# shrubb/latent-pose-reenactment

Hardware: AMD Instinct MI355X
Metric: train-step images/sec at 256x256 bs=8 (higher is better)
Workload: dtype mixed 16-bit MFMA operands, fp32 accumulate, fp32 activations / weights / optimizer state; 1 GPU; default.yaml meta-training step (configs[2]): ResNeXt50 identity encoder over 8 frames + MobileNetV2 pose encoder (both trained, forward + backward on hand-written gfx950 kernels), G, D with the 98000x512 label embedding, VGG19/VGGFace/featmat/adversarial/dis_embed/dice criterions, Adam, EMA; image_size=256, per_gpu_batch=8, global_batch=8, parallelism=dp1, precision_mode=default assignment (LP_PREC=f16), padding=zero, launch_mode=hipgraph

## Files before the change

include/lp_hip.h:

```cpp
#ifndef LP_HIP_H
#define LP_HIP_H
#include <stdint.h>
#ifdef __cplusplus
extern "C" {
#endif

#define LP_OK 0
#define LP_ERR_ARG (-1)
#define LP_ERR_UNSUPPORTED (-2)
#define LP_ERR_HIP (-3)

#define LP_PREC_BF16 0
#define LP_PREC_BF16X3 1
#define LP_PREC_F16 2

const char* lp_last_error(void);
int lp_abi_version(void);

int lp_pack_weights(const float* w, uint16_t* hi, uint16_t* lo, int Cout, int Cin, int T, int RowsP, int ColsP, int mode, int f16,
                    void* stream);
int lp_pack_desc_bytes(void);
int lp_pack_weights_batch(const void* table, int num_entries, long long total_chunks, void* stream);
int lp_pack_pair_desc_bytes(void);
int lp_pack_weights_pairs(const void* table, int num_entries, long long total_tiles, void* stream);
// ... 89 lines not shown
                    int frozen_stats, float* amax_slots, void* stream);

long long lp_bn_train_stats_workspace_bytes(long long P, int C);
int lp_bn_train_stats(const float* y, const float* gamma, const float* beta, float eps, float momentum, float* running_mean,
                      float* running_var, float* mean, float* rstd, float* scale, float* shift, float* workspace,
                      long long P, int C, void* stream);

int lp_gconv16_fwd(const uint16_t* a_hi, const uint16_t* a_lo, const uint16_t* w_hi, const uint16_t* w_lo, float* y, const float* alpha2,
                   int N, int H, int W, int C, int CP, int prec, float* amax_slots, void* stream);
int lp_gconv16_fwd_stats(const uint16_t* a_hi, const uint16_t* a_lo, const uint16_t* w_hi, const uint16_t* w_lo, float* y, const float* alpha2,
                         int N, int H, int W, int C, int CP, int prec, float* amax_slots, float* stats, long long stats_capacity_floats,
                         int* stats_rows, void* stream);
int lp_gconv16_fwd_planes(const uint16_t* a_hi, const uint16_t* a_lo, const uint16_t* w_hi, const uint16_t* w_lo, float* y, uint16_t* o_hi,
                          uint16_t* o_lo, const float* alpha2, int N, int H, int W, int C, int CP, int group_size, int prec, float* amax_slots,
                          float* stats, long long stats_capacity_floats, int* stats_rows, void* stream);
long long lp_gconv_wgrad_workspace_bytes(int C, int splits);
int lp_gconv16_wgrad(const uint16_t* a_hi, const uint16_t* a_lo, const uint16_t* dy_hi, const uint16_t* dy_lo, float* dw, float* workspace,
                     int N, int H, int W, int C, int group_size, int splits, int prec, const float* out_scale, void* stream);
int lp_pack_grouped(const float* w, uint16_t* hi, uint16_t* lo, int C, int group_size, int CP, int mode, int f16, void* stream);
int lp_im2col_planes(const float* x, uint16_t* hi, uint16_t* lo, int N, int C, int H, int W, int ksize, int stride, int pad, int prec,
                     void* stream);
int lp_bn_relu_maxpool_fwd(const float* y, const float* scale, const float* shift, float* out, uint16_t* hi, uint16_t* lo,
                           unsigned char* idx, int N, int H, int W, int C, int prec, void* stream);
int lp_maxpool_bwd(const float* dout, const unsigned char* idx, float* dA, int N, int H, int W, int C, void* stream);
int lp_bn_add_act(const float* y, const float* scale, const float* shift, const float* res, const float* res_scale, const float* res_shift,
                  float* out, uint16_t* hi, uint16_t* lo, long long P, int C, int relu, int prec, void* stream);
int lp_bn_add_act_planes(const float* y, const float* scale, const float* shift, const uint16_t* res_hi, const uint16_t* res_lo, float* out,
                         uint16_t* hi, uint16_t* lo, long long P, int C, int relu, int prec, void* stream);
int lp_bn_add_act16(const uint16_t* y16, const float* scale, const float* shift, const float* res, const float* res_scale,
                    const float* res_shift, float* out, uint16_t* hi, long long P, int C, int relu, void* stream);
// ... 147 lines not shown
```

latent_pose_reenactment_amd/_lib.py:

```python
import ctypes
import os

import torch

_HERE = os.path.dirname(os.path.abspath(__file__))
LIB_PATH = os.environ.get('LP_LIB_OVERRIDE') or os.path.join(_HERE, 'liblp_hip.so')

PREC_BF16 = 0
PREC_BF16X3 = 1
PREC_F16 = 2

_vp, _i, _f, _ll = ctypes.c_void_p, ctypes.c_int, ctypes.c_float, ctypes.c_longlong

SIGNATURES = {
    'lp_last_error': (ctypes.c_char_p, []),
    'lp_abi_version': (_i, []),
    'lp_pack_weights': (_i, [_vp, _vp, _vp, _i, _i, _i, _i, _i, _i, _i, _vp]),
    'lp_pack_desc_bytes': (_i, []),
    'lp_pack_weights_batch': (_i, [_vp, _i, _ll, _vp]),
    'lp_pack_pair_desc_bytes': (_i, []),
    'lp_pack_weights_pairs': (_i, [_vp, _i, _ll, _vp]),
    'lp_act_pack': (_i, [_vp, _vp, _vp, _i, _vp, _vp, _i, _i, _i, _i, _vp, _vp, _i, _i, _vp, _vp]),
    'lp_amax_slots': (_i, []),
    'lp_amax_slot_stride': (_i, []),
    'lp_amax_blocks': (_i, []),
    'lp_amax_partial': (_i, [_vp, _ll, _vp, _vp]),
    'lp_conv16_fwd': (_i, [_vp] * 9 + [_i] * 11 + [_vp, _vp, _vp, _i, _vp, _ll, _vp, _vp]),
    'lp_conv16_fwd_workspace_bytes': (_ll, [_i] * 5),
    'lp_conv16_fwd_stats': (_i, [_vp] * 9 + [_i] * 11 + [_vp, _vp, _vp, _i, _vp, _ll, _vp, _vp, _ll, _vp, _vp]),
    'lp_conv16_stats_floats': (_ll, [_i] * 4),
    'lp_norm_stats_finalize': (_i, [_vp, _i, _vp, _vp, _i, _f, _f, _vp, _vp, _vp, _vp, _vp, _vp, _i, _i, _vp]),
    'lp_gconv16_fwd_stats': (_i, [_vp] * 6 + [_i] * 6 + [_vp, _vp, _ll, _vp, _vp]),
    'lp_gconv16_fwd_planes': (_i, [_vp] * 8 + [_i] * 7 + [_vp, _vp, _ll, _vp, _vp]),
    'lp_conv_wgrad_workspace_bytes': (_ll, [_i, _i, _i, _i]),
    'lp_conv16_wgrad': (_i, [_vp] * 6 + [_i] * 9 + [_vp, _i, _vp, _vp, _vp, _vp]),
    'lp_conv_wgrad_dot_blocks': (_i, [_i] * 3),
    'lp_thin_conv_supported': (_i, [_i] * 4),
    'lp_thin_conv_fwd': (_i, [_vp] * 6 + [_i] * 9 + [_vp, _i, _vp]),
    'lp_thin_conv_emits_planes': (_i, [_i] * 5),
    'lp_thin_wgrad_supported': (_i, [_i] * 5),
    'lp_thin_wgrad_has_dbias': (_i, [_i] * 2),
    'lp_thin_wgrad': (_i, [_vp] * 6 + [_i] * 8 + [_vp, _vp]),
    'lp_linear_fwd': (_i, [_vp, _vp, _vp, _vp, _vp, _i, _i, _i, _vp]),
    'lp_linear_bwd_workspace_bytes': (_ll, [_i, _i, _i]),
    'lp_linear_bwd': (_i, [_vp] * 8 + [_i, _i, _i, _vp]),
    'lp_grid_crop_fwd': (_i, [_vp, _vp, _vp, _i, _i, _i, _i, _i, _i, _vp]),
    'lp_grid_crop_bwd': (_i, [_vp, _vp, _vp, _i, _i, _i, _i, _i, _i, _vp]),
    'lp_stem_conv_s2': (_i, [_vp, _vp, _vp, _i, _i, _i, _i, _vp]),
# ... 108 lines not shown
_lib = None


class LpError(RuntimeError):
    pass


def lib():
    global _lib
    if _lib is None:
        if not os.path.exists(LIB_PATH):
            raise LpError(f'{LIB_PATH} is missing: run `python -m latent_pose_reenactment_amd.build` '
                          '(or __graft_entry__.build()); there is no fallback path')
        l = ctypes.CDLL(LIB_PATH)
        for name, (res, args) in SIGNATURES.items():
            fn = getattr(l, name)
            fn.restype, fn.argtypes = res, args
        _lib = l
    return _lib


def check(rc, what):
    if rc != 0:
        msg = lib().lp_last_error()
        raise LpError(f'{what} failed (rc={rc}): {msg.decode() if msg else ""}')
```

latent_pose_reenactment_amd/csrc/gconv_rows.hip:

```cpp
#include "lp_common.h"
#include "conv_common.h"
#include "lp_hip.h"
#include "lp_internal.h"
#include <stdlib.h>

#if defined(__HIP_DEVICE_COMPILE__)
#pragma clang attribute push(__attribute__((target("no-packed-fp32-ops"))), apply_to = function)
#endif

static __device__ __attribute__((aligned(64))) unsigned int gr_zero_page[16];

static __device__ __forceinline__ void gr_barrier() {
    __builtin_amdgcn_fence(__ATOMIC_RELEASE, "workgroup");
    __builtin_amdgcn_s_barrier();
    __builtin_amdgcn_fence(__ATOMIC_ACQUIRE, "workgroup");
}
static __device__ __forceinline__ float gr_shfl_xor(float v, int lane, int o) {
    return __builtin_bit_cast(float, __builtin_amdgcn_ds_bpermute((lane ^ o) << 2, __builtin_bit_cast(int, v)));
}

struct GconvRowsParams {
    const uint16_t* a_hi; const uint16_t* a_lo; const uint16_t* w_hi; const uint16_t* w_lo;
    float* y; uint16_t* o_hi; uint16_t* o_lo; const float* alpha2; float* amax; float* stats;
    int N, H, W, C, CP;
    int tiles_x, tiles_y, ntiles;
    int nblk, wgs, xcd;
};

namespace gr {
constexpr int TH = 4, TW = 16, HH = TH + 2, HW = TW + 2, HALO_PX = HH * HW;
constexpr int PIECES = (HALO_PX * 128 + 1023) / 1024;
constexpr int PLANE = PIECES * 1024;
constexpr int KIT = (PIECES + 3) / 4;
__host__ __device__ constexpr int key(int hp) { return ((hp >> 1) & 3) << 1; }
}

template <int PREC>
__global__ __launch_bounds__(256, PREC == LP_PREC_BF16X3 ? 2 : 4) void gconv_rows_kernel(GconvRowsParams p) {
    using namespace gr;
    constexpr bool SPLIT = (PREC == LP_PREC_BF16X3), F16 = (PREC == LP_PREC_F16);
    constexpr int BUF = PLANE * (SPLIT ? 2 : 1);
    extern __shared__ __attribute__((aligned(16))) unsigned char smem[];

    const int lane = (int)threadIdx.x & 63;
    const int wave = __builtin_amdgcn_readfirstlane((int)threadIdx.x >> 6);
    const int kb = lane >> 4, px = lane & 15;

    int blk, t0, tstep, tend;
    {
        const int id = (int)blockIdx.x;
        if (p.xcd) {
            const int x = id & 7, j = id >> 3, per = (p.ntiles + 7) >> 3;
            blk = j % p.nblk;
            tstep = p.wgs >> 3;
// ... 17 lines not shown
        wlo[s] = (s16x8_t){0, 0, 0, 0, 0, 0, 0, 0};
        if (tap < 9) {
            const size_t off = ((size_t)tap * p.CP + co0 + 16 * wave + px) * 64 + 16 * wave + 8 * (kb & 1);
            whi[s] = *(const s16x8_t*)(p.w_hi + off);
            if (SPLIT) wlo[s] = *(const s16x8_t*)(p.w_lo + off);
        }
    }
    const float alpha = p.alpha2 ? *p.alpha2 : 1.f;

    int r_off[TH][5];
#pragma unroll
    for (int s = 0; s < 5; ++s) {
        const int tap = min(2 * s + (lane >> 5), 8);
#pragma unroll
        for (int r = 0; r < TH; ++r) {
            const int hp = (r + tap / 3) * HW + px + tap % 3;
            r_off[r][s] = hp * 128 + (((2 * wave + (kb & 1)) ^ key(hp)) << 4);
        }
    }

    int d_hy[KIT], d_hx[KIT], d_c[KIT];
#pragma unroll
    for (int k = 0; k < KIT; ++k) {
        const int hp = (4 * k + wave) * 8 + (lane >> 3);
        d_hy[k] = hp < HALO_PX ? hp / HW : -(1 << 20);
        d_hx[k] = hp % HW;
        d_c[k] = co0 + (((lane & 7) ^ key(hp)) << 3);
    }
    const uint16_t* zero16 = (const uint16_t*)gr_zero_page;
    const unsigned lds0 = (unsigned)__builtin_amdgcn_readfirstlane((int)(unsigned)(uintptr_t)smem);
    auto decode = [&](int t, int& n, int& y0, int& x0) {
        x0 = (t % p.tiles_x) * TW; t /= p.tiles_x;
        y0 = (t % p.tiles_y) * TH; n = t / p.tiles_y;
    };
    auto issue = [&](int t, int buf) {
        int n, y0, x0;
        decode(t, n, y0, x0);
#pragma unroll
        for (int k = 0; k < KIT; ++k) {
            const int q = 4 * k + wave;
            if (q < PIECES) {
                const int iy = y0 - 1 + d_hy[k], ix = x0 - 1 + d_hx[k];
                const bool ok = iy >= 0 && iy < p.H && ix >= 0 && ix < p.W;
                const size_t off = ok ? ((size_t)(n * p.H + iy) * p.W + ix) * p.C + d_c[k] : 0;
                const unsigned d = lds0 + (unsigned)(buf * BUF + q * 1024);
                lp_glds16(ok ? (p.a_hi + off) : zero16, d);
                if (SPLIT) lp_glds16(ok ? (p.a_lo + off) : zero16, d + PLANE);
            }
        }
    };

    float am = 0.f;
    issue(t0, 0);
    int buf = 0;
    for (int t = t0; t < tend; t += tstep, buf ^= 1) {
        lp_wait_vm0();
        gr_barrier();
// ... 28 lines not shown
            const int oy = y0 + r, ox = x0 + px;
            float4 v;
            v.x = fmaf(acc[0], alpha, 0.f); v.y = fmaf(acc[1], alpha, 0.f); v.z = fmaf(acc[2], alpha, 0.f); v.w = fmaf(acc[3], alpha, 0.f);
            if (p.stats) {
                const float o4[4] = {v.x, v.y, v.z, v.w};
#pragma unroll
                for (int k = 0; k < 4; ++k)
#pragma unroll
                    for (int j = 0; j < 4; ++j) {
                        const float xv = __builtin_bit_cast(float, __builtin_amdgcn_ds_bpermute(((lane & 48) | (4 * k + (px & 3))) << 2, __builtin_bit_cast(int, o4[j])));
                        if (r == 0 && k == 0) st_ref[j] = xv;
                        const float d = xv - st_ref[j];
                        st_d[j] += d; st_q[j] = fmaf(d, d, st_q[j]);
                    }
            }
            if (oy < p.H && ox < p.W) {
                const size_t e = (((size_t)n * p.H + oy) * p.W + ox) * p.C + co0 + 16 * wave + 4 * kb;
                if (p.y) *(float4*)(p.y + e) = v;
                am = lp_amax4(am, v);
                if (p.o_hi) {
                    const float o[4] = {v.x, v.y, v.z, v.w};
                    ushort4 oh, ol;
                    uint16_t* ohp = (uint16_t*)&oh; uint16_t* olp = (uint16_t*)&ol;
#pragma unroll
                    for (int j = 0; j < 4; ++j) {
                        ohp[j] = lp_f32_to_op16<F16>(o[j]);
                        if (SPLIT) olp[j] = lp_f32_to_op16<false>(o[j] - lp_op16_to_f32<false>(ohp[j]));
                    }
                    *(ushort4*)(p.o_hi + e) = oh;
                    if (SPLIT) *(ushort4*)(p.o_lo + e) = ol;
                }
            }
// ... 2 lines not shown
            float cnt = 16.f, mean[4], m2[4];
#pragma unroll
            for (int j = 0; j < 4; ++j) { mean[j] = st_ref[j] + st_d[j] / cnt; m2[j] = fmaxf(st_q[j] - st_d[j] * st_d[j] / cnt, 0.f); }
#pragma unroll
            for (int o = 1; o < 4; o <<= 1) {
#pragma unroll
                for (int j = 0; j < 4; ++j) {
                    const float mb = gr_shfl_xor(mean[j], lane, o), qb = gr_shfl_xor(m2[j], lane, o);
                    const float d = mb - mean[j];
                    mean[j] = fmaf(d, 0.5f, mean[j]); m2[j] += qb + d * d * (cnt * 0.5f);
                }
                cnt *= 2.f;
            }
            if (px == 0) {
                const int ty = y0 >> 2;
                const int rb = ((n * (p.tiles_y >> 2) + (ty >> 2)) * p.tiles_x + (x0 >> 4)) * 4 + (ty & 3);
                float* o = p.stats + ((size_t)rb * p.C + co0 + 16 * wave + 4 * kb) * 3;
#pragma unroll
                for (int j = 0; j < 4; ++j) { o[j * 3 + 0] = cnt; o[j * 3 + 1] = mean[j]; o[j * 3 + 2] = m2[j]; }
            }
        }
    }
    if (p.amax) lp_amax_commit(am, p.amax, blockIdx.x);
}

#if defined(__HIP_DEVICE_COMPILE__)
#pragma clang attribute pop
#endif

int lp_gconv_rows_launch(Conv16Params& c, int group_size, int prec, hipStream_t s) {
    static const int mode = getenv("LP_GCONV_ROWS") ? atoi(getenv("LP_GCONV_ROWS")) : 1;
    static const int wgs_cap = getenv("LP_GCONV_ROWS_WGS") ? atoi(getenv("LP_GCONV_ROWS_WGS")) : 0;
    if (mode == 0 || !(group_size == 4 || group_size == 8 || group_size == 16)) return 0;
    if (prec != LP_PREC_BF16 && prec != LP_PREC_BF16X3 && prec != LP_PREC_F16) return 0;
    const bool exact = (c.W % gr::TW == 0) && (c.H % gr::TH == 0);
    if (mode != 2 && !exact) return 0;
    const bool patches = (c.W % 16 == 0) && (c.H % 16 == 0);
    if (c.stats && !patches && (c.H * c.W) % 64 == 0) return 0;
    GconvRowsParams p;
    p.a_hi = c.a_hi; p.a_lo = c.a_lo; p.w_hi = c.w_hi; p.w_lo = c.w_lo; p.y = c.y; p.o_hi = c.o_hi; p.o_lo = c.o_lo; p.alpha2 = c.alpha2; p.amax = c.amax;
    p.N = c.N; p.H = c.H; p.W = c.W; p.C = c.Cout; p.CP = c.CoutP;
    p.tiles_x = (c.W + gr::TW - 1) / gr::TW; p.tiles_y = (c.H + gr::TH - 1) / gr::TH; p.ntiles = c.N * p.tiles_x * p.tiles_y;
    p.nblk = c.Cout / 64;
    c.stats_rows = 0;
    if (c.stats) {
        const long long rows = (long long)c.N * (c.H * c.W / 64);
        if (patches && rows * c.Cout * 3 <= c.stats_cap) c.stats_rows = c.H * c.W / 64; else c.stats = nullptr;
    }
    p.stats = c.stats;
    const int occ = prec == LP_PREC_BF16X3 ? 2 : 4;
    static int cus = 0;
    if (!cus) { int dev = 0; if (hipGetDevice(&dev) != hipSuccess || hipDeviceGetAttribute(&cus, hipDeviceAttributeMultiprocessorCount, dev) != hipSuccess || cus < 1) cus = 256; }
    int wgs = (cus * occ + p.nblk - 1) / p.nblk;
    if (wgs_cap > 0 && wgs > wgs_cap) wgs = wgs_cap;
    if (wgs > p.ntiles) wgs = p.ntiles;
    p.xcd = (wgs >= 8 && p.ntiles >= 16) ? 1 : 0;
    if (p.xcd) wgs &= ~7;
    p.wgs = wgs;
    const dim3 grid((unsigned)(p.nblk * wgs));
    const size_t lds = 2 * gr::PLANE * (prec == LP_PREC_BF16X3 ? 2 : 1);
    if (prec == LP_PREC_BF16X3) hipLaunchKernelGGL(gconv_rows_kernel<LP_PREC_BF16X3>, grid, dim3(256), lds, s, p);
    else if (prec == LP_PREC_F16) hipLaunchKernelGGL(gconv_rows_kernel<LP_PREC_F16>, grid, dim3(256), lds, s, p);
    else hipLaunchKernelGGL(gconv_rows_kernel<LP_PREC_BF16>, grid, dim3(256), lds, s, p);
    const int rc = lp_check_launch("gconv_rows");
    return rc ? rc : 1;
}
```

latent_pose_reenactment_amd/embedders/resnext_hip.py:

```python
import os

import torch

from latent_pose_reenactment_amd import hipops as ops
from latent_pose_reenactment_amd import streams as _streams
from latent_pose_reenactment_amd._lib import PREC_BF16X3, PREC_F16


class _BN:
    __slots__ = ('mean', 'rstd', 'scale', 'shift')

    def __init__(self, mean, rstd, scale, shift):
        self.mean, self.rstd, self.scale, self.shift = mean, rstd, scale, shift


def supported(n: int, h: int, w: int) -> bool:
    return h % 32 == 0 and w % 32 == 0 and h >= 128 and w >= 128 and n % 4 == 0 and n >= 8


Y16 = os.environ.get('LP_E_Y16', '1') != '0'
RES16 = os.environ.get('LP_E_RES16', '1') != '0'
MASK16 = os.environ.get('LP_E_MASK16', '1') != '0'


# ... 23 lines not shown
def _bn_relu_planes(y, st, prec):
    if isinstance(y, ops.Act16):
        return ops.bn_act16(y, st.scale, st.shift)
    return ops.act_pack(y, pro=4, scale=st.scale, shift=st.shift, prec=prec)


def bn_state(y, st, gamma, beta, m, counters):
    if m.track_running_stats:
        counters.append(m.num_batches_tracked)
    rm, rv = (m.running_mean, m.running_var) if m.track_running_stats else (None, None)
    if st is not None:
        return _BN(*ops.norm_stats_finalize(st, 1, gamma.shape[0], gamma, beta, m.eps, running_mean=rm, running_var=rv, momentum=m.momentum))
    if isinstance(y, ops.Act16):
        y = ops.y16_to_f32(y)
    return _BN(*ops.bn_train_stats(y, gamma, beta, rm, rv, m.momentum, m.eps))


def _wgrad1x1(a16, d16, prec, bias_grad=False):
    return ops.conv_wgrad16(ops.flat16(a16), ops.flat16(d16), ksize=1, prec=prec, bias_grad=bias_grad, kind='wgrad1x1')


class ResNeXtFunction(torch.autograd.Function):

    @staticmethod
    def forward(ctx, net, x, *params):
        prec = net.prec
        train = net.training
        need_grad = any(ctx.needs_input_grad[2:])
        if ctx.needs_input_grad[1]:
            raise RuntimeError('the HIP encoder does not differentiate with respect to its input frames (detach them)')
# ... 34 lines not shown
            y16 = Y16 and p1 == p2 == p3 == PREC_F16
            assert not (y16 and nprec != PREC_F16), 'an fp16 block must be followed by fp16 blocks (lp_bn_add_act16 writes fp16 planes)'
            xin, xin16 = out, out16
            _, h, w, _ = xin16.hi.shape
            y1, cs = _conv1x1(xin16, packs[bname + '.conv1.weight'][0], p1, stats=True, y16=y16)
            y1 = _yview(y1, (n, h, w, width))
            st1 = bn(y1, bname + '.bn1', cs)
            a1 = _bn_relu_planes(y1, st1, p2)
            if stride == 1:
                if y16:
                    _, y2, cs = ops.gconv16(a1, packs[bname + '.conv2.weight'][0], prec=p2, stats=True, want_y=False, out16=True)
                else:
                    y2, cs = ops.gconv16(a1, packs[bname + '.conv2.weight'][0], prec=p2, stats=True)
                ho, wo = h, w
            else:
                y2, cs = ops.subsample2(ops.gconv16(a1, packs[bname + '.conv2.weight'][0], prec=p2)), None
                ho, wo = y2.shape[1], y2.shape[2]
            st2 = bn(y2, bname + '.bn2', cs)
            a2 = _bn_relu_planes(y2, st2, p3)
            y3, cs = _conv1x1(a2, packs[bname + '.conv3.weight'][0], p3, stats=True, y16=y16)
            y3 = _yview(y3, (n, ho, wo, cout))
            st3 = bn(y3, bname + '.bn3', cs)
            xd16 = yd = std = None
            if down:
                xd16 = ops.subsample2_16(xin16) if stride == 2 else xin16
                yd, cs = _conv1x1(xd16, packs[bname + '.downsample.0.weight'][0], p1, stats=True)
                yd = yd.view(n, ho, wo, cout)
                std = bn(yd, bname + '.downsample.1', cs)
                need_f32 = bi + 1 >= nblk or not (net._hip_blocks[bi + 1][5] or planes_res[bi + 1])
                out, out16 = ops.bn_add_act(y3, st3.scale, st3.shift, yd, std.scale, std.shift, relu=True, prec=nprec, want_out=need_f32 or not MASK16)
            elif planes_res[bi]:
# ... 47 lines not shown
            else:
                grads[key] = fn(*operands)

        p16, (hl, wl, cl), (fh, fw) = ctx.head
        dl16 = ops.act_pack(d_logits.contiguous().view(1, fh, fw, -1), prec=prec, grad=True)
        dw, db = ops.conv_wgrad16(p16, dl16, ksize=1, prec=prec, bias_grad=True)
        grads['fc.weight'], grads['fc.bias'] = dw.view(par['fc.weight'].shape), db
        d_pooled = ops.conv16(dl16, packs['fc.weight'][1], ksize=1, prec=prec).view(n, cl)
        d_out = ops.spatial_mean_bwd(d_pooled, hl, wl)
        for (bname, cin, width, cout, stride, down), sv in zip(reversed(net._hip_blocks), reversed(ctx.blocks)):
            xin16, y1, st1, a1, y2, st2, a2, y3, st3, xd16, yd, std, out, (h, w, ho, wo), (p1, p2, p3) = sv
            d16, g = bn_bwd(d_out, y3, st3, bname + '.bn3', p3, mask_mode=2, mask_src=out, want_g=not down)
            wgrad(bname + '.conv3.weight', lambda a, d, k=bname + '.conv3.weight', p=p3: _wgrad1x1(a, d, p).view(par[k].shape), a2, d16)
            dA2 = _conv1x1(d16, packs[bname + '.conv3.weight'][1], p3).view(n, ho, wo, width)
            d16, _ = bn_bwd(dA2, y2, st2, bname + '.bn2', p2)
            if stride == 2:
                d16 = ops.zero_stuff2_16(d16, h, w)
            cg = par[bname + '.conv2.weight'].shape[1]
            wgrad(bname + '.conv2.weight', lambda a, d, cg=cg, p=p2: ops.gconv_wgrad16(a, d, cg, prec=p), a1, d16)
            dA1 = ops.gconv16(d16, packs[bname + '.conv2.weight'][1], prec=p2)
            d16, _ = bn_bwd(dA1, y1, st1, bname + '.bn1', p1)
            wgrad(bname + '.conv1.weight', lambda a, d, k=bname + '.conv1.weight', p=p1: _wgrad1x1(a, d, p).view(par[k].shape), xin16, d16)
            if down:
                dd16, _ = bn_bwd(d_out, yd, std, bname + '.downsample.1', p1, mask_mode=2, mask_src=out)
                wgrad(bname + '.downsample.0.weight', lambda a, d, k=bname + '.downsample.0.weight', p=p1: _wgrad1x1(a, d, p).view(par[k].shape), xd16, dd16)
                d_xd = _conv1x1(dd16, packs[bname + '.downsample.0.weight'][1], p1)
                if stride == 2:
                    d_xin = _conv1x1(d16, packs[bname + '.conv1.weight'][1], p1).view(n, h, w, cin)
                    ops.add_strided2(d_xin, d_xd.view(n, ho, wo, cin))
                else:
                    d_xin = _conv1x1(d16, packs[bname + '.conv1.weight'][1], p1, res=d_xd).view(n, h, w, cin)
            else:
                d_xin = _conv1x1(d16, packs[bname + '.conv1.weight'][1], p1, res=g).view(n, h, w, cin)
            d_out = d_xin
        prec = net.prec
# ... 11 lines not shown
```

latent_pose_reenactment_amd/hipops.py:

```python
import os
from typing import NamedTuple, Optional, Tuple

import torch

from . import _lib
from ._lib import PREC_BF16, PREC_BF16X3, PREC_F16, check
from .dataloaders.synthetic_voxceleb2_stickmen import PARTS

Tensor = torch.Tensor


def _stream():
    return torch.cuda.current_stream().cuda_stream


PROFILE = None


class _Timed:
    def __init__(self, kind, flops, tag=None, nbytes=0.0, mm=1):
        self.mm = mm
        self.rw = tuple(nbytes) if isinstance(nbytes, tuple) else None
        self.kind, self.flops, self.tag, self.nbytes = kind, flops, tag, (sum(nbytes) if isinstance(nbytes, tuple) else nbytes)

# ... 1820 lines not shown
                                     mask_mode, mptr, _p(g), float(act_hi), int(frozen), _p(_amax_attach(dx, amax)), _stream()),
          'lp_norm_act_bwd')
    return dx, dgb[0], dgb[1], g


def pack_grouped(w: Tensor, mode: int, prec: int) -> WeightPack:
    _chk(w, 'w')
    c, cg = w.shape[0], w.shape[1]
    cp = _round_up(c, 128)
    hi = torch.empty((9, cp, 64), dtype=torch.int16, device=w.device)
    lo = torch.empty_like(hi) if prec == PREC_BF16X3 else None
    check(_lib.lib().lp_pack_grouped(w.data_ptr(), hi.data_ptr(), _p(lo), c, cg, cp, mode, _f16(prec), _stream()), 'lp_pack_grouped')
    return WeightPack(hi, lo, c, cg, cp, 64, 9)


def gconv16(a: Act16, pack: WeightPack, *, prec: int, amax: bool = False, stats: bool = False, want_y: bool = True, out16: bool = False):
    n, h, w = a.nhw
    c = a.c
    assert c == pack.rows and a.hi.shape[3] == c, (a.hi.shape, pack.rows)
    assert want_y or (out16 and not amax)
    dev = a.hi.device
    y = torch.empty((n, h, w, c), dtype=torch.float32, device=dev) if want_y else None
    o_hi = o_lo = None
    if out16:
        o_hi, o_lo = _alloc16(n, h, w, c, prec, dev)
    slots = _amax_attach(y, amax and prec == PREC_F16) if y is not None else None
    st_buf, st_rows, st_cap = None, None, 0
    if stats:
        import ctypes
        st_cap = _lib.lib().lp_conv16_stats_floats(n, h, w, c)
        st_buf = torch.empty(st_cap, dtype=torch.float32, device=dev)
        st_rows = ctypes.c_int(0)
    pl = 4 if prec == PREC_BF16X3 else 2
    nbytes = n * h * w * c * (pl + (4 if want_y else 0) + (pl if out16 else 0)) + pack.hi.numel() * pl
    with _Timed('gconv', 2.0 * n * h * w * c * pack.cols * 9, (n, h, w, pack.cols, c, 3, 0, 0), nbytes, mm=3 if prec == PREC_BF16X3 else 1):
        check(_lib.lib().lp_gconv16_fwd_planes(a.hi.data_ptr(), _p(a.lo), pack.hi.data_ptr(), _p(pack.lo), _p(y), _p(o_hi), _p(o_lo), _p(a.inv),
                                               n, h, w, c, pack.rows_p, pack.cols, prec, _p(slots), _p(st_buf), st_cap,
                                               None if st_rows is None else ctypes.addressof(st_rows), _stream()), 'lp_gconv16_fwd')
    out = (y,) if not out16 else (y, Act16(o_hi, o_lo, c, None))
    if stats:
        out = out + ((ConvStats(st_buf, st_rows.value, n) if st_rows.value > 0 else None),)
    return out[0] if len(out) == 1 else out


def bn_act16(y16: Act16, scale: Tensor, shift: Tensor, relu: bool = True) -> Act16:
    c = y16.c
    assert y16.lo is None and y16.inv is None and y16.hi.shape[-1] == c and c % 8 == 0
    hi = torch.empty_like(y16.hi)
    check(_lib.lib().lp_bn_act16(y16.hi.data_ptr(), scale.data_ptr(), shift.data_ptr(), hi.data_ptr(), y16.hi.numel() // c, c, int(relu),
                                 _stream()), 'lp_bn_act16')
    return Act16(hi, None, c, None)


# ... 267 lines not shown
```

Before: 204.9 images/s.

## Add native stride-2 grouped conv forward and polyphase dgrad for ResNeXt

Adds a stride-2 variant of the row-tiled grouped 3x3 conv kernel that computes only the subsampled outputs, with fused BN stats, instead of running a full-resolution conv and subsampling afterwards. It also adds a polyphase stride-2 data-gradient kernel that reads the low-resolution gradient directly, so the zero-stuffed full-resolution gradient is no longer convolved. The point is to remove the wasted MACs (about 3/4) and memory traffic in the stride-2 blocks of the ResNeXt encoder. The cost is more kernel code and a halo layout with even/odd column splitting, plus lower occupancy bounds for the S=2 kernel.

```diff
diff --git a/include/lp_hip.h b/include/lp_hip.h
--- a/include/lp_hip.h
+++ b/include/lp_hip.h
@@ -127,6 +127,12 @@
 int lp_gconv16_fwd_planes(const uint16_t* a_hi, const uint16_t* a_lo, const uint16_t* w_hi, const uint16_t* w_lo, float* y, uint16_t* o_hi,
                           uint16_t* o_lo, const float* alpha2, int N, int H, int W, int C, int CP, int group_size, int prec, float* amax_slots,
                           float* stats, long long stats_capacity_floats, int* stats_rows, void* stream);
+int lp_gconv16_s2_covered(int H, int W, int group_size);
+int lp_gconv16_s2_fwd_planes(const uint16_t* a_hi, const uint16_t* a_lo, const uint16_t* w_hi, const uint16_t* w_lo, float* y, uint16_t* o_hi,
+                             uint16_t* o_lo, const float* alpha2, int N, int H, int W, int C, int CP, int group_size, int prec,
+                             float* amax_slots, float* stats, long long stats_capacity_floats, int* stats_rows, void* stream);
+int lp_gconv16_s2_dgrad(const uint16_t* d_hi, const uint16_t* d_lo, const uint16_t* w_hi, const uint16_t* w_lo, float* dx, const float* alpha2,
+                        int N, int H, int W, int C, int CP, int group_size, int prec, float* amax_slots, void* stream);
 long long lp_gconv_wgrad_workspace_bytes(int C, int splits);
 int lp_gconv16_wgrad(const uint16_t* a_hi, const uint16_t* a_lo, const uint16_t* dy_hi, const uint16_t* dy_lo, float* dw, float* workspace,
                      int N, int H, int W, int C, int group_size, int splits, int prec, const float* out_scale, void* stream);
diff --git a/latent_pose_reenactment_amd/_lib.py b/latent_pose_reenactment_amd/_lib.py
--- a/latent_pose_reenactment_amd/_lib.py
+++ b/latent_pose_reenactment_amd/_lib.py
@@ -32,6 +32,9 @@
     'lp_norm_stats_finalize': (_i, [_vp, _i, _vp, _vp, _i, _f, _f, _vp, _vp, _vp, _vp, _vp, _vp, _i, _i, _vp]),
     'lp_gconv16_fwd_stats': (_i, [_vp] * 6 + [_i] * 6 + [_vp, _vp, _ll, _vp, _vp]),
     'lp_gconv16_fwd_planes': (_i, [_vp] * 8 + [_i] * 7 + [_vp, _vp, _ll, _vp, _vp]),
+    'lp_gconv16_s2_covered': (_i, [_i] * 3),
+    'lp_gconv16_s2_fwd_planes': (_i, [_vp] * 8 + [_i] * 7 + [_vp, _vp, _ll, _vp, _vp]),
+    'lp_gconv16_s2_dgrad': (_i, [_vp] * 6 + [_i] * 7 + [_vp, _vp]),
     'lp_conv_wgrad_workspace_bytes': (_ll, [_i, _i, _i, _i]),
     'lp_conv16_wgrad': (_i, [_vp] * 6 + [_i] * 9 + [_vp, _i, _vp, _vp, _vp, _vp]),
     'lp_conv_wgrad_dot_blocks': (_i, [_i] * 3),
@@ -170,6 +173,8 @@
                           '(or __graft_entry__.build()); there is no fallback path')
         l = ctypes.CDLL(LIB_PATH)
         for name, (res, args) in SIGNATURES.items():
+            if os.environ.get('LP_LIB_OVERRIDE') and not hasattr(l, name):
+                continue
             fn = getattr(l, name)
             fn.restype, fn.argtypes = res, args
         _lib = l
diff --git a/latent_pose_reenactment_amd/csrc/gconv_rows.hip b/latent_pose_reenactment_amd/csrc/gconv_rows.hip
--- a/latent_pose_reenactment_amd/csrc/gconv_rows.hip
+++ b/latent_pose_reenactment_amd/csrc/gconv_rows.hip
@@ -23,21 +23,28 @@
     const uint16_t* a_hi; const uint16_t* a_lo; const uint16_t* w_hi; const uint16_t* w_lo;
     float* y; uint16_t* o_hi; uint16_t* o_lo; const float* alpha2; float* amax; float* stats;
     int N, H, W, C, CP;
+    int Ho, Wo;
     int tiles_x, tiles_y, ntiles;
     int nblk, wgs, xcd;
 };
 
 namespace gr {
-constexpr int TH = 4, TW = 16, HH = TH + 2, HW = TW + 2, HALO_PX = HH * HW;
-constexpr int PIECES = (HALO_PX * 128 + 1023) / 1024;
-constexpr int PLANE = PIECES * 1024;
-constexpr int KIT = (PIECES + 3) / 4;
+constexpr int TH = 4, TW = 16;
+template <int S> struct Geo {
+    static constexpr int HH = S * (TH - 1) + 3, HW = S * (TW - 1) + 3, HALO_PX = HH * HW;
+    static constexpr int EV = TW + 1;
+    static constexpr int PIECES = (HALO_PX * 128 + 1023) / 1024;
+    static constexpr int PLANE = PIECES * 1024;
+    static constexpr int KIT = (PIECES + 3) / 4;
+};
 __host__ __device__ constexpr int key(int hp) { return ((hp >> 1) & 3) << 1; }
 }
 
-template <int PREC>
-__global__ __launch_bounds__(256, PREC == LP_PREC_BF16X3 ? 2 : 4) void gconv_rows_kernel(GconvRowsParams p) {
+template <int PREC, int S>
+__global__ __launch_bounds__(256, (PREC == LP_PREC_BF16X3 ? 2 : 4) / S) void gconv_rows_kernel(GconvRowsParams p) {
     using namespace gr;
+    using G = Geo<S>;
+    constexpr int HW = G::HW, HALO_PX = G::HALO_PX, PIECES = G::PIECES, PLANE = G::PLANE, KIT = G::KIT;
     constexpr bool SPLIT = (PREC == LP_PREC_BF16X3), F16 = (PREC == LP_PREC_F16);
     constexpr int BUF = PLANE * (SPLIT ? 2 : 1);
     extern __shared__ __attribute__((aligned(16))) unsigned char smem[];
@@ -85,7 +92,8 @@
         const int tap = min(2 * s + (lane >> 5), 8);
 #pragma unroll
         for (int r = 0; r < TH; ++r) {
-            const int hp = (r + tap / 3) * HW + px + tap % 3;
+            const int dy = tap / 3, dx = tap % 3;
+            const int hp = S == 1 ? (r + dy) * HW + px + dx : (2 * r + dy) * HW + (dx == 1 ? G::EV + px : px + (dx >> 1));
             r_off[r][s] = hp * 128 + (((2 * wave + (kb & 1)) ^ key(hp)) << 4);
         }
     }
@@ -95,7 +103,7 @@
     for (int k = 0; k < KIT; ++k) {
         const int hp = (4 * k + wave) * 8 + (lane >> 3);
         d_hy[k] = hp < HALO_PX ? hp / HW : -(1 << 20);
-        d_hx[k] = hp % HW;
+        d_hx[k] = S == 1 ? hp % HW : (hp % HW < G::EV ? 2 * (hp % HW) : 2 * (hp % HW - G::EV) + 1);
         d_c[k] = co0 + (((lane & 7) ^ key(hp)) << 3);
     }
     const uint16_t* zero16 = (const uint16_t*)gr_zero_page;
@@ -111,7 +119,7 @@
         for (int k = 0; k < KIT; ++k) {
             const int q = 4 * k + wave;
             if (q < PIECES) {
-                const int iy = y0 - 1 + d_hy[k], ix = x0 - 1 + d_hx[k];
+                const int iy = S * y0 - 1 + d_hy[k], ix = S * x0 - 1 + d_hx[k];
                 const bool ok = iy >= 0 && iy < p.H && ix >= 0 && ix < p.W;
                 const size_t off = ok ? ((size_t)(n * p.H + iy) * p.W + ix) * p.C + d_c[k] : 0;
                 const unsigned d = lds0 + (unsigned)(buf * BUF + q * 1024);
@@ -170,8 +178,8 @@
                         st_d[j] += d; st_q[j] = fmaf(d, d, st_q[j]);
                     }
             }
-            if (oy < p.H && ox < p.W) {
-                const size_t e = (((size_t)n * p.H + oy) * p.W + ox) * p.C + co0 + 16 * wave + 4 * kb;
+            if (oy < p.Ho && ox < p.Wo) {
+                const size_t e = (((size_t)n * p.Ho + oy) * p.Wo + ox) * p.C + co0 + 16 * wave + 4 * kb;
                 if (p.y) *(float4*)(p.y + e) = v;
                 am = lp_amax4(am, v);
                 if (p.o_hi) {
@@ -204,10 +212,162 @@
             }
             if (px == 0) {
                 const int ty = y0 >> 2;
-                const int rb = ((n * (p.tiles_y >> 2) + (ty >> 2)) * p.tiles_x + (x0 >> 4)) * 4 + (ty & 3);
+                const int rb = S == 1 ? ((n * (p.tiles_y >> 2) + (ty >> 2)) * p.tiles_x + (x0 >> 4)) * 4 + (ty & 3) : t;
                 float* o = p.stats + ((size_t)rb * p.C + co0 + 16 * wave + 4 * kb) * 3;
 #pragma unroll
                 for (int j = 0; j < 4; ++j) { o[j * 3 + 0] = cnt; o[j * 3 + 1] = mean[j]; o[j * 3 + 2] = m2[j]; }
+            }
+        }
+    }
+    if (p.amax) lp_amax_commit(am, p.amax, blockIdx.x);
+}
+
+struct GconvS2DgradParams {
+    const uint16_t* d_hi; const uint16_t* d_lo; const uint16_t* w_hi; const uint16_t* w_lo;
+    float* dx; const float* alpha2; float* amax;
+    int N, H, W, Ho, Wo, C, CP;
+    int tiles_x, tiles_y, ntiles;
+    int nblk, wgs, xcd;
+};
+
+namespace gd {
+constexpr int TH = 4, TW = 16, HH = TH + 1, HW = TW + 1, HALO_PX = HH * HW;
+constexpr int PIECES = (HALO_PX * 128 + 1023) / 1024;
+constexpr int PLANE = PIECES * 1024;
+constexpr int KIT = (PIECES + 3) / 4;
+}
+
+template <int PREC>
+__global__ __launch_bounds__(256, PREC == LP_PREC_BF16X3 ? 2 : 4) void gconv_rows_s2_dgrad_kernel(GconvS2DgradParams p) {
+    using namespace gd;
+    constexpr bool SPLIT = (PREC == LP_PREC_BF16X3), F16 = (PREC == LP_PREC_F16);
+    constexpr int BUF = PLANE * (SPLIT ? 2 : 1);
+    extern __shared__ __attribute__((aligned(16))) unsigned char smem[];
+
+    const int lane = (int)threadIdx.x & 63;
+    const int wave = __builtin_amdgcn_readfirstlane((int)threadIdx.x >> 6);
+    const int kb = lane >> 4, px = lane & 15;
+
+    int blk, t0, tstep, tend;
+    {
+        const int id = (int)blockIdx.x;
+        if (p.xcd) {
+            const int x = id & 7, j = id >> 3, per = (p.ntiles + 7) >> 3;
+            blk = j % p.nblk;
+            tstep = p.wgs >> 3;
+            t0 = x * per + j / p.nblk;
+            tend = min(x * per + per, p.ntiles);
+        } else {
+            blk = id % p.nblk;
+            tstep = p.wgs;
+            t0 = id / p.nblk;
+            tend = p.ntiles;
+        }
+    }
+    if (t0 >= tend) return;
+    const int co0 = blk * 64;
+
+    s16x8_t whi[5], wlo[5];
+#pragma unroll
+    for (int s = 0; s < 5; ++s) {
+        const int tap = 2 * s + (lane >> 5);
+        whi[s] = (s16x8_t){0, 0, 0, 0, 0, 0, 0, 0};
+        wlo[s] = (s16x8_t){0, 0, 0, 0, 0, 0, 0, 0};
+        if (tap < 9) {
+            const size_t off = ((size_t)tap * p.CP + co0 + 16 * wave + px) * 64 + 16 * wave + 8 * (kb & 1);
+            whi[s] = *(const s16x8_t*)(p.w_hi + off);
+            if (SPLIT) wlo[s] = *(const s16x8_t*)(p.w_lo + off);
+        }
+    }
+    const float alpha = p.alpha2 ? *p.alpha2 : 1.f;
+
+    int r_off[HH][2];
+#pragma unroll
+    for (int hy = 0; hy < HH; ++hy)
+#pragma unroll
+        for (int ex = 0; ex < 2; ++ex) {
+            const int hp = hy * HW + px + ex;
+            r_off[hy][ex] = hp * 128 + (((2 * wave + (kb & 1)) ^ gr::key(hp)) << 4);
+        }
+
+    int d_hy[KIT], d_hx[KIT], d_c[KIT];
+#pragma unroll
+    for (int k = 0; k < KIT; ++k) {
+        const int hp = (4 * k + wave) * 8 + (lane >> 3);
+        d_hy[k] = hp < HALO_PX ? hp / HW : (1 << 20);
+        d_hx[k] = hp % HW;
+        d_c[k] = co0 + (((lane & 7) ^ gr::key(hp)) << 3);
+    }
+    const uint16_t* zero16 = (const uint16_t*)gr_zero_page;
+    const unsigned lds0 = (unsigned)__builtin_amdgcn_readfirstlane((int)(unsigned)(uintptr_t)smem);
+    auto decode = [&](int t, int& n, int& y0, int& x0) {
+        x0 = (t % p.tiles_x) * TW; t /= p.tiles_x;
+        y0 = (t % p.tiles_y) * TH; n = t / p.tiles_y;
+    };
+    auto issue = [&](int t, int buf) {
+        int n, y0, x0;
+        decode(t, n, y0, x0);
+#pragma unroll
+        for (int k = 0; k < KIT; ++k) {
+            const int q = 4 * k + wave;
+            if (q < PIECES) {
+                const int sy = y0 + d_hy[k], sx = x0 + d_hx[k];
+                const bool ok = sy < p.Ho && sx < p.Wo;
+                const size_t off = ok ? ((size_t)(n * p.Ho + sy) * p.Wo + sx) * p.C + d_c[k] : 0;
+                const unsigned d = lds0 + (unsigned)(buf * BUF + q * 1024);
+                lp_glds16(ok ? (p.d_hi + off) : zero16, d);
+                if (SPLIT) lp_glds16(ok ? (p.d_lo + off) : zero16, d + PLANE);
+            }
+        }
+    };
+
+    float am = 0.f;
+    issue(t0, 0);
+    int buf = 0;
+    for (int t = t0; t < tend; t += tstep, buf ^= 1) {
+        lp_wait_vm0();
+        gr_barrier();
+        if (t + tstep < tend) issue(t + tstep, buf ^ 1);
+        int n, y0, x0;
+        decode(t, n, y0, x0);
+        const unsigned char* Hb = smem + buf * BUF;
+#pragma unroll
+        for (int a = 0; a < TH; ++a) {
+            int lhalf = lane >> 5;
+            asm volatile("" : "+v"(lhalf));
+            s16x8_t fh[2][2], fl[2][2];
+#pragma unroll
+            for (int ey = 0; ey < 2; ++ey)
+#pragma unroll
+                for (int ex = 0; ex < 2; ++ex) {
+                    fh[ey][ex] = *(const s16x8_t*)(Hb + r_off[a + ey][ex]);
+                    if (SPLIT) fl[ey][ex] = *(const s16x8_t*)(Hb + PLANE + r_off[a + ey][ex]);
+                }
+#pragma unroll
+            for (int ph = 0; ph < 4; ++ph) {
+                const int pa = ph >> 1, pb = ph & 1;
+                f32x4_t acc = (f32x4_t){0.f, 0.f, 0.f, 0.f};
+#pragma unroll
+                for (int tap = 0; tap < 9; ++tap) {
+                    const int dy = tap / 3, dx = tap % 3;
+                    if ((dy == 1) != (pa == 0) || (dx == 1) != (pb == 0)) continue;
+                    const int ey = dy == 2, ex = dx == 2, s = tap >> 1, h = tap & 1;
+                    const s16x8_t zero = (s16x8_t){0, 0, 0, 0, 0, 0, 0, 0};
+                    const s16x8_t mh = (lhalf == h) ? whi[s] : zero;
+                    if (SPLIT) {
+                        const s16x8_t ml = (lhalf == h) ? wlo[s] : zero;
+                        acc = mfma16t<false>(mh, fl[ey][ex], acc);
+                        acc = mfma16t<false>(ml, fh[ey][ex], acc);
+                    }
+                    acc = mfma16t<F16>(mh, fh[ey][ex], acc);
+                }
+                const int iy = 2 * (y0 + a) + pa, ix = 2 * (x0 + px) + pb;
+                float4 v;
+                v.x = fmaf(acc[0], alpha, 0.f); v.y = fmaf(acc[1], alpha, 0.f); v.z = fmaf(acc[2], alpha, 0.f); v.w = fmaf(acc[3], alpha, 0.f);
+                if (iy < p.H && ix < p.W) {
+                    *(float4*)(p.dx + (((size_t)n * p.H + iy) * p.W + ix) * p.C + co0 + 16 * wave + 4 * kb) = v;
+                    am = lp_amax4(am, v);
+                }
             }
         }
     }
@@ -218,9 +378,26 @@
 #pragma clang attribute pop
 #endif
 
+static int gr_mode() {
+    static const int mode = getenv("LP_GCONV_ROWS") ? atoi(getenv("LP_GCONV_ROWS")) : 1;
+    return mode;
+}
+
+static int gr_workgroups(int nblk, int ntiles, int occ, int& xcd) {
+    static const int wgs_cap = getenv("LP_GCONV_ROWS_WGS") ? atoi(getenv("LP_GCONV_ROWS_WGS")) : 0;
+    static int cus = 0;
+    if (!cus) { int dev = 0; if (hipGetDevice(&dev) != hipSuccess || hipDeviceGetAttribute(&cus, hipDeviceAttributeMultiprocessorCount, dev) != hipSuccess || cus < 1) cus = 256; }
+    int wgs = (cus * occ + nblk - 1) / nblk;
+    if (wgs_cap > 0 && wgs > wgs_cap) wgs = wgs_cap;
+    if (wgs > ntiles) wgs = ntiles;
+    xcd = (wgs >= 8 && ntiles >= 16) ? 1 : 0;
+    if (xcd) wgs &= ~7;
+    return wgs;
+}
+
 int lp_gconv_rows_launch(Conv16Params& c, int group_size, int prec, hipStream_t s) {
-    static const int mode = getenv("LP_GCONV_ROWS") ? atoi(getenv("LP_GCONV_ROWS")) : 1;
-    static const int wgs_cap = getenv("LP_GCONV_ROWS_WGS") ? atoi(getenv("LP_GCONV_ROWS_WGS")) : 0;
+    using G = gr::Geo<1>;
+    const int mode = gr_mode();
     if (mode == 0 || !(group_size == 4 || group_size == 8 || group_size == 16)) return 0;
     if (prec != LP_PREC_BF16 && prec != LP_PREC_BF16X3 && prec != LP_PREC_F16) return 0;
     const bool exact = (c.W % gr::TW == 0) && (c.H % gr::TH == 0);
@@ -229,7 +406,7 @@
     if (c.stats && !patches && (c.H * c.W) % 64 == 0) return 0;
     GconvRowsParams p;
     p.a_hi = c.a_hi; p.a_lo = c.a_lo; p.w_hi = c.w_hi; p.w_lo = c.w_lo; p.y = c.y; p.o_hi = c.o_hi; p.o_lo = c.o_lo; p.alpha2 = c.alpha2; p.amax = c.amax;
-    p.N = c.N; p.H = c.H; p.W = c.W; p.C = c.Cout; p.CP = c.CoutP;
+    p.N = c.N; p.H = c.H; p.W = c.W; p.Ho = c.H; p.Wo = c.W; p.C = c.Cout; p.CP = c.CoutP;
     p.tiles_x = (c.W + gr::TW - 1) / gr::TW; p.tiles_y = (c.H + gr::TH - 1) / gr::TH; p.ntiles = c.N * p.tiles_x * p.tiles_y;
     p.nblk = c.Cout / 64;
     c.stats_rows = 0;
@@ -238,20 +415,96 @@
         if (patches && rows * c.Cout * 3 <= c.stats_cap) c.stats_rows = c.H * c.W / 64; else c.stats = nullptr;
     }
     p.stats = c.stats;
-    const int occ = prec == LP_PREC_BF16X3 ? 2 : 4;
-    static int cus = 0;
-    if (!cus) { int dev = 0; if (hipGetDevice(&dev) != hipSuccess || hipDeviceGetAttribute(&cus, hipDeviceAttributeMultiprocessorCount, dev) != hipSuccess || cus < 1) cus = 256; }
-    int wgs = (cus * occ + p.nblk - 1) / p.nblk;
-    if (wgs_cap > 0 && wgs > wgs_cap) wgs = wgs_cap;
-    if (wgs > p.ntiles) wgs = p.ntiles;
-    p.xcd = (wgs >= 8 && p.ntiles >= 16) ? 1 : 0;
-    if (p.xcd) wgs &= ~7;
-    p.wgs = wgs;
-    const dim3 grid((unsigned)(p.nblk * wgs));
-    const size_t lds = 2 * gr::PLANE * (prec == LP_PREC_BF16X3 ? 2 : 1);
-    if (prec == LP_PREC_BF16X3) hipLaunchKernelGGL(gconv_rows_kernel<LP_PREC_BF16X3>, grid, dim3(256), lds, s, p);
-    else if (prec == LP_PREC_F16) hipLaunchKernelGGL(gconv_rows_kernel<LP_PREC_F16>, grid, dim3(256), lds, s, p);
-    else hipLaunchKernelGGL(gconv_rows_kernel<LP_PREC_BF16>, grid, dim3(256), lds, s, p);
+    p.wgs = gr_workgroups(p.nblk, p.ntiles, prec == LP_PREC_BF16X3 ? 2 : 4, p.xcd);
+    const dim3 grid((unsigned)(p.nblk * p.wgs));
+    const size_t lds = 2 * G::PLANE * (prec == LP_PREC_BF16X3 ? 2 : 1);
+    if (prec == LP_PREC_BF16X3) hipLaunchKernelGGL((gconv_rows_kernel<LP_PREC_BF16X3, 1>), grid, dim3(256), lds, s, p);
+    else if (prec == LP_PREC_F16) hipLaunchKernelGGL((gconv_rows_kernel<LP_PREC_F16, 1>), grid, dim3(256), lds, s, p);
+    else hipLaunchKernelGGL((gconv_rows_kernel<LP_PREC_BF16, 1>), grid, dim3(256), lds, s, p);
     const int rc = lp_check_launch("gconv_rows");
     return rc ? rc : 1;
 }
+
+
+extern "C" int lp_gconv16_s2_covered(int H, int W, int group_size) {
+    const int mode = gr_mode();
+    if (mode == 0 || !(group_size == 4 || group_size == 8 || group_size == 16)) return 0;
+    if (H < 2 || W < 2 || (H & 1) || (W & 1)) return 0;
+    if (mode != 2 && ((W / 2) % gr::TW || (H / 2) % gr::TH)) return 0;
+    return 1;
+}
+
+static int gr_s2_check(int N, int H, int W, int C, int CP, int group_size, int prec) {
+    if ((C & 63) || CP % 128 || CP < C) return lp_set_error(LP_ERR_UNSUPPORTED, "lp_gconv16_s2: C must be a multiple of 64, CP of 128");
+    if (prec != LP_PREC_BF16 && prec != LP_PREC_BF16X3 && prec != LP_PREC_F16) return lp_set_error(LP_ERR_ARG, "lp_gconv16_s2: unknown precision mode");
+    if (N < 1 || !lp_gconv16_s2_covered(H, W, group_size))
+        return lp_set_error(LP_ERR_UNSUPPORTED, "lp_gconv16_s2: shape not covered (lp_gconv16_s2_covered): use the stride-1 route");
+    if ((long long)N * H * W * C >= (1ll << 31)) return lp_set_error(LP_ERR_UNSUPPORTED, "lp_gconv16_s2: tensor too large");
+    return LP_OK;
+}
+
+extern "C" int lp_gconv16_s2_fwd_planes(const uint16_t* a_hi, const uint16_t* a_lo, const uint16_t* w_hi, const uint16_t* w_lo, float* y,
+                                        uint16_t* o_hi, uint16_t* o_lo, const float* alpha2, int N, int H, int W, int C, int CP, int group_size,
+                                        int prec, float* amax_slots, float* stats, long long stats_capacity_floats, int* stats_rows,
+                                        void* stream) {
+    using G = gr::Geo<2>;
+    if (stats_rows) *stats_rows = 0;
+    if (stats && !stats_rows) return lp_set_error(LP_ERR_ARG, "lp_gconv16_s2_fwd: stats needs stats_rows");
+    if (!a_hi || !w_hi || (!y && !o_hi)) return lp_set_error(LP_ERR_ARG, "lp_gconv16_s2_fwd: null pointer");
+    if (o_hi && prec == LP_PREC_BF16X3 && !o_lo) return lp_set_error(LP_ERR_ARG, "lp_gconv16_s2_fwd: bf16x3 output planes need lo");
+    if (prec == LP_PREC_BF16X3 && (!w_lo || !a_lo)) return lp_set_error(LP_ERR_ARG, "lp_gconv16_s2_fwd: bf16x3 needs the lo planes");
+    int rc = gr_s2_check(N, H, W, C, CP, group_size, prec);
+    if (rc) return rc;
+    GconvRowsParams p;
+    p.a_hi = a_hi; p.a_lo = a_lo; p.w_hi = w_hi; p.w_lo = w_lo; p.y = y; p.o_hi = o_hi; p.o_lo = o_lo; p.alpha2 = alpha2; p.amax = amax_slots;
+    p.N = N; p.H = H; p.W = W; p.Ho = H / 2; p.Wo = W / 2; p.C = C; p.CP = CP;
+    p.tiles_x = (p.Wo + gr::TW - 1) / gr::TW; p.tiles_y = (p.Ho + gr::TH - 1) / gr::TH; p.ntiles = N * p.tiles_x * p.tiles_y;
+    p.nblk = C / 64;
+    p.stats = nullptr;
+    if (stats && p.Wo % gr::TW == 0 && p.Ho % gr::TH == 0 && (long long)p.ntiles * C * 3 <= stats_capacity_floats) {
+        p.stats = stats;
+        *stats_rows = p.tiles_x * p.tiles_y;
+    }
+    const bool split = prec == LP_PREC_BF16X3;
+    p.wgs = gr_workgroups(p.nblk, p.ntiles, split ? 1 : 2, p.xcd);
+    const dim3 grid((unsigned)(p.nblk * p.wgs));
+    const size_t lds = 2 * G::PLANE * (split ? 2 : 1);
+    const void* kern = split ? (const void*)gconv_rows_kernel<LP_PREC_BF16X3, 2>
+                             : prec == LP_PREC_F16 ? (const void*)gconv_rows_kernel<LP_PREC_F16, 2> : (const void*)gconv_rows_kernel<LP_PREC_BF16, 2>;
+    static int attr_dev[3] = {-1, -1, -1};
+    int dev = 0;
+    if (hipGetDevice(&dev) != hipSuccess) return lp_set_error(LP_ERR_HIP, "hipGetDevice failed");
+    if (attr_dev[prec] != dev) {
+        if (hipFuncSetAttribute(kern, hipFuncAttributeMaxDynamicSharedMemorySize, 160 * 1024) != hipSuccess)
+            return lp_set_error(LP_ERR_HIP, "hipFuncSetAttribute failed");
+        attr_dev[prec] = dev;
+    }
+    hipStream_t s = (hipStream_t)stream;
+    if (split) hipLaunchKernelGGL((gconv_rows_kernel<LP_PREC_BF16X3, 2>), grid, dim3(256), lds, s, p);
+    else if (prec == LP_PREC_F16) hipLaunchKernelGGL((gconv_rows_kernel<LP_PREC_F16, 2>), grid, dim3(256), lds, s, p);
+    else hipLaunchKernelGGL((gconv_rows_kernel<LP_PREC_BF16, 2>), grid, dim3(256), lds, s, p);
+    return lp_check_launch("gconv_rows_s2");
+}
+
+extern "C" int lp_gconv16_s2_dgrad(const uint16_t* d_hi, const uint16_t* d_lo, const uint16_t* w_hi, const uint16_t* w_lo, float* dx,
+                                   const float* alpha2, int N, int H, int W, int C, int CP, int group_size, int prec, float* amax_slots,
+                                   void* stream) {
+    if (!d_hi || !w_hi || !dx) return lp_set_error(LP_ERR_ARG, "lp_gconv16_s2_dgrad: null pointer");
+    if (prec == LP_PREC_BF16X3 && (!w_lo || !d_lo)) return lp_set_error(LP_ERR_ARG, "lp_gconv16_s2_dgrad: bf16x3 needs the lo planes");
+    int rc = gr_s2_check(N, H, W, C, CP, group_size, prec);
+    if (rc) return rc;
+    GconvS2DgradParams p;
+    p.d_hi = d_hi; p.d_lo = d_lo; p.w_hi = w_hi; p.w_lo = w_lo; p.dx = dx; p.alpha2 = alpha2; p.amax = amax_slots;
+    p.N = N; p.H = H; p.W = W; p.Ho = H / 2; p.Wo = W / 2; p.C = C; p.CP = CP;
+    p.tiles_x = (p.Wo + gd::TW - 1) / gd::TW; p.tiles_y = (p.Ho + gd::TH - 1) / gd::TH; p.ntiles = N * p.tiles_x * p.tiles_y;
+    p.nblk = C / 64;
+    const bool split = prec == LP_PREC_BF16X3;
+    p.wgs = gr_workgroups(p.nblk, p.ntiles, split ? 2 : 4, p.xcd);
+    const dim3 grid((unsigned)(p.nblk * p.wgs));
+    const size_t lds = 2 * gd::PLANE * (split ? 2 : 1);
+    hipStream_t s = (hipStream_t)stream;
+    if (split) hipLaunchKernelGGL(gconv_rows_s2_dgrad_kernel<LP_PREC_BF16X3>, grid, dim3(256), lds, s, p);
+    else if (prec == LP_PREC_F16) hipLaunchKernelGGL(gconv_rows_s2_dgrad_kernel<LP_PREC_F16>, grid, dim3(256), lds, s, p);
+    else hipLaunchKernelGGL(gconv_rows_s2_dgrad_kernel<LP_PREC_BF16>, grid, dim3(256), lds, s, p);
+    return lp_check_launch("gconv_rows_s2_dgrad");
+}
diff --git a/latent_pose_reenactment_amd/embedders/resnext_hip.py b/latent_pose_reenactment_amd/embedders/resnext_hip.py
--- a/latent_pose_reenactment_amd/embedders/resnext_hip.py
+++ b/latent_pose_reenactment_amd/embedders/resnext_hip.py
@@ -61,6 +61,25 @@
     if isinstance(y, ops.Act16):
         y = ops.y16_to_f32(y)
     return _BN(*ops.bn_train_stats(y, gamma, beta, rm, rv, m.momentum, m.eps))
+
+
+def _s2_covered(h, w, cg):
+    f = getattr(ops, 'gconv16_s2_covered', None)
+    return f is not None and f(h, w, cg)
+
+
+def _gconv_s2_fwd(a1, pack, prec, cg):
+    _, h, w, _ = a1.hi.shape
+    if _s2_covered(h, w, cg):
+        return ops.gconv16(a1, pack, prec=prec, stats=True, stride=2)
+    return ops.subsample2(ops.gconv16(a1, pack, prec=prec)), None
+
+
+def _gconv_s2_dgrad(dlow, dfull, pack, prec, cg):
+    _, h, w, _ = dfull.hi.shape
+    if _s2_covered(h, w, cg):
+        return ops.gconv16(dlow, pack, prec=prec, stride=2, out_hw=(h, w))
+    return ops.gconv16(dfull, pack, prec=prec)
 
 
 def _wgrad1x1(a16, d16, prec, bias_grad=False):
@@ -125,7 +144,7 @@
                     y2, cs = ops.gconv16(a1, packs[bname + '.conv2.weight'][0], prec=p2, stats=True)
                 ho, wo = h, w
             else:
-                y2, cs = ops.subsample2(ops.gconv16(a1, packs[bname + '.conv2.weight'][0], prec=p2)), None
+                y2, cs = _gconv_s2_fwd(a1, packs[bname + '.conv2.weight'][0], p2, par[bname + '.conv2.weight'].shape[1])
                 ho, wo = y2.shape[1], y2.shape[2]
             st2 = bn(y2, bname + '.bn2', cs)
             a2 = _bn_relu_planes(y2, st2, p3)
@@ -203,11 +222,15 @@
             wgrad(bname + '.conv3.weight', lambda a, d, k=bname + '.conv3.weight', p=p3: _wgrad1x1(a, d, p).view(par[k].shape), a2, d16)
             dA2 = _conv1x1(d16, packs[bname + '.conv3.weight'][1], p3).view(n, ho, wo, width)
             d16, _ = bn_bwd(dA2, y2, st2, bname + '.bn2', p2)
+            cg = par[bname + '.conv2.weight'].shape[1]
+            dlow = d16
             if stride == 2:
                 d16 = ops.zero_stuff2_16(d16, h, w)
-            cg = par[bname + '.conv2.weight'].shape[1]
             wgrad(bname + '.conv2.weight', lambda a, d, cg=cg, p=p2: ops.gconv_wgrad16(a, d, cg, prec=p), a1, d16)
-            dA1 = ops.gconv16(d16, packs[bname + '.conv2.weight'][1], prec=p2)
+            if stride == 2:
+                dA1 = _gconv_s2_dgrad(dlow, d16, packs[bname + '.conv2.weight'][1], p2, cg)
+            else:
+                dA1 = ops.gconv16(d16, packs[bname + '.conv2.weight'][1], prec=p2)
             d16, _ = bn_bwd(dA1, y1, st1, bname + '.bn1', p1)
             wgrad(bname + '.conv1.weight', lambda a, d, k=bname + '.conv1.weight', p=p1: _wgrad1x1(a, d, p).view(par[k].shape), xin16, d16)
             if down:
diff --git a/latent_pose_reenactment_amd/hipops.py b/latent_pose_reenactment_amd/hipops.py
--- a/latent_pose_reenactment_amd/hipops.py
+++ b/latent_pose_reenactment_amd/hipops.py
@@ -1858,12 +1858,41 @@
     return WeightPack(hi, lo, c, cg, cp, 64, 9)
 
 
-def gconv16(a: Act16, pack: WeightPack, *, prec: int, amax: bool = False, stats: bool = False, want_y: bool = True, out16: bool = False):
+def gconv16_s2_covered(h: int, w: int, group_size: int) -> bool:
+    fn = getattr(_lib.lib(), 'lp_gconv16_s2_covered', None)
+    return bool(fn(h, w, group_size)) if fn is not None else False
+
+
+def _gconv16_s2_dgrad(d: Act16, pack: WeightPack, out_hw, prec: int, amax: bool):
+    n, hs, ws_ = d.nhw
+    h, w = out_hw
+    c = d.c
+    assert c == pack.rows and d.hi.shape[3] == c and (hs, ws_) == (h // 2, w // 2) and h % 2 == 0 and w % 2 == 0, (d.hi.shape, out_hw)
+    dx = torch.empty((n, h, w, c), dtype=torch.float32, device=d.hi.device)
+    slots = _amax_attach(dx, amax and prec == PREC_F16)
+    pl = 4 if prec == PREC_BF16X3 else 2
+    nbytes = n * hs * ws_ * c * pl + n * h * w * c * 4 + pack.hi.numel() * pl
+    with _Timed('gconv', 2.0 * n * hs * ws_ * c * pack.cols * 9, (n, h, w, pack.cols, c, 3, 0, 0), nbytes, mm=3 if prec == PREC_BF16X3 else 1):
+        check(_lib.lib().lp_gconv16_s2_dgrad(d.hi.data_ptr(), _p(d.lo), pack.hi.data_ptr(), _p(pack.lo), dx.data_ptr(), _p(d.inv), n, h, w, c,
+                                             pack.rows_p, pack.cols, prec, _p(slots), _stream()), 'lp_gconv16_s2_dgrad')
+    return dx
+
+
+def gconv16(a: Act16, pack: WeightPack, *, prec: int, amax: bool = False, stats: bool = False, want_y: bool = True, out16: bool = False,
+            stride: int = 1, out_hw=None):
+    assert stride in (1, 2) and (out_hw is None or stride == 2)
+    if out_hw is not None:
+        assert want_y and not stats and not out16
+        return _gconv16_s2_dgrad(a, pack, out_hw, prec, amax)
     n, h, w = a.nhw
     c = a.c
     assert c == pack.rows and a.hi.shape[3] == c, (a.hi.shape, pack.rows)
     assert want_y or (out16 and not amax)
     dev = a.hi.device
+    hin, win = h, w
+    if stride == 2:
+        assert h % 2 == 0 and w % 2 == 0, (h, w)
+        h, w = h // 2, w // 2
     y = torch.empty((n, h, w, c), dtype=torch.float32, device=dev) if want_y else None
     o_hi = o_lo = None
     if out16:
@@ -1876,11 +1905,13 @@
         st_buf = torch.empty(st_cap, dtype=torch.float32, device=dev)
         st_rows = ctypes.c_int(0)
     pl = 4 if prec == PREC_BF16X3 else 2
-    nbytes = n * h * w * c * (pl + (4 if want_y else 0) + (pl if out16 else 0)) + pack.hi.numel() * pl
-    with _Timed('gconv', 2.0 * n * h * w * c * pack.cols * 9, (n, h, w, pack.cols, c, 3, 0, 0), nbytes, mm=3 if prec == PREC_BF16X3 else 1):
-        check(_lib.lib().lp_gconv16_fwd_planes(a.hi.data_ptr(), _p(a.lo), pack.hi.data_ptr(), _p(pack.lo), _p(y), _p(o_hi), _p(o_lo), _p(a.inv),
-                                               n, h, w, c, pack.rows_p, pack.cols, prec, _p(slots), _p(st_buf), st_cap,
-                                               None if st_rows is None else ctypes.addressof(st_rows), _stream()), 'lp_gconv16_fwd')
+    nbytes = n * hin * win * c * pl + n * h * w * c * ((4 if want_y else 0) + (pl if out16 else 0)) + pack.hi.numel() * pl
+    fwd = _lib.lib().lp_gconv16_fwd_planes if stride == 1 else _lib.lib().lp_gconv16_s2_fwd_planes
+    with _Timed('gconv', 2.0 * n * h * w * c * pack.cols * 9, (n, h, w, pack.cols, c, 3, 0, 0), nbytes,
+                mm=3 if prec == PREC_BF16X3 else 1):
+        check(fwd(a.hi.data_ptr(), _p(a.lo), pack.hi.data_ptr(), _p(pack.lo), _p(y), _p(o_hi), _p(o_lo), _p(a.inv),
+                  n, hin, win, c, pack.rows_p, pack.cols, prec, _p(slots), _p(st_buf), st_cap,
+                  None if st_rows is None else ctypes.addressof(st_rows), _stream()), 'lp_gconv16_fwd')
     out = (y,) if not out16 else (y, Act16(o_hi, o_lo, c, None))
     if stats:
         out = out + ((ConvStats(st_buf, st_rows.value, n) if st_rows.value > 0 else None),)
```

Result: no change. 206.6 images/s, median of 3 (+0.8%).
